# EugenHotaj/pytorch-generative

Hardware: NVIDIA H100
Metric: images/sec training step (ImageGPT CIFAR-10 32x32) (higher is better)
Workload: dtype bf16

## Files before the change

### pytorch_generative_b200/csrc/pg_attention.cu

```cuda
#include <stdlib.h>
#include <type_traits>

#include "../../include/pg_b200.h"
#include "pg_common.cuh"

namespace {

constexpr int MAX_S = 1024;
constexpr int MAX_D = 128;

struct AttnArgs {
  const bf16 *q, *k, *v, *o, *d_o;
  bf16 *out, *dq, *dk_out, *dv_out;
  int64_t ld_q, ld_k, ld_v, ld_o, ld_do, ld_dq, ld_dk, ld_dv;
  float* lse;
  const float* lse_in;
  float* delta;
  int N, S, H, dk, dv, strict;
  float scale;
};

__global__ void __launch_bounds__(128) attn_fwd_simt(const AttnArgs a) {
  extern __shared__ float sm[];
  const int lane = threadIdx.x & 31, w = threadIdx.x >> 5;
// ... 6 lines not shown
  const int h = (int)((gw / a.S) % a.H);
  const int n = (int)(gw / ((long long)a.S * a.H));
  const size_t row0 = (size_t)n * a.S;
  for (int d = lane; d < a.dk; d += 32) qs[d] = __bfloat162float(a.q[(row0 + i) * a.ld_q + h * a.dk + d]);
  __syncwarp();
  const int nkeys = a.strict ? i : i + 1;
  float m = -INFINITY;
  for (int j = lane; j < nkeys; j += 32) {
    const bf16* kr = a.k + (row0 + j) * a.ld_k + h * a.dk;
    float s = 0.f;
    for (int d = 0; d < a.dk; ++d) s = fmaf(qs[d], __bfloat162float(kr[d]), s);
    s *= a.scale;
    sc[j] = s;
    m = fmaxf(m, s);
  }
  m = warp_max(m);
  float l = 0.f;
  for (int j = lane; j < nkeys; j += 32) {
    const float p = __expf(sc[j] - m);
    sc[j] = p;
    l += p;
  }
  l = warp_sum(l);
  __syncwarp();
  const float inv = nkeys > 0 ? 1.f / l : 0.f;
  for (int d = lane; d < a.dv; d += 32) {
    float acc = 0.f;
    for (int j = 0; j < nkeys; ++j) acc = fmaf(sc[j], __bfloat162float(a.v[(row0 + j) * a.ld_v + h * a.dv + d]), acc);
    a.out[(row0 + i) * a.ld_o + h * a.dv + d] = __float2bfloat16(acc * inv);
  }
  if (lane == 0 && a.lse) a.lse[((size_t)n * a.H + h) * a.S + i] = nkeys > 0 ? m + __logf(l) : 0.f;
}

__global__ void attn_delta_kernel(const AttnArgs a) {
  const int lanes_per = a.dv / 8;
  const long long total = (long long)a.N * a.S * a.H * lanes_per;
  for (long long idx = (long long)blockIdx.x * blockDim.x + threadIdx.x; idx < total;
       idx += (long long)gridDim.x * blockDim.x) {
    const int sub = (int)(idx % lanes_per);
    const long long rh = idx / lanes_per;
    const int h = (int)(rh % a.H);
    const long long row = rh / a.H;
    const uint4 x = *reinterpret_cast<const uint4*>(a.d_o + row * a.ld_do + h * a.dv + sub * 8);
    const uint4 y = *reinterpret_cast<const uint4*>(a.o + row * a.ld_o + h * a.dv + sub * 8);
    const uint32_t xw[4] = {x.x, x.y, x.z, x.w}, yw[4] = {y.x, y.y, y.z, y.w};
    float s = 0.f;
#pragma unroll
    for (int t = 0; t < 4; ++t) {
      const float2 p = unpack_bf16x2(xw[t]), q = unpack_bf16x2(yw[t]);
      s = fmaf(p.x, q.x, fmaf(p.y, q.y, s));
    }
    for (int o = lanes_per >> 1; o > 0; o >>= 1) s += __shfl_xor_sync(0xffffffffu, s, o);
    if (sub == 0) {
      const int n = (int)(row / a.S), i = (int)(row % a.S);
      a.delta[((size_t)n * a.H + h) * a.S + i] = s;
    }
  }
}

__global__ void attn_delta_generic_kernel(const AttnArgs a) {
  const int lane = threadIdx.x & 31;
  const long long gw = ((long long)blockIdx.x * blockDim.x + threadIdx.x) >> 5;
  const long long total = (long long)a.N * a.H * a.S;
  if (gw >= total) return;
  const int i = (int)(gw % a.S);
  const int h = (int)((gw / a.S) % a.H);
  const int n = (int)(gw / ((long long)a.S * a.H));
  const size_t row = (size_t)n * a.S + i;
  float s = 0.f;
  for (int d = lane; d < a.dv; d += 32)
    s += __bfloat162float(a.d_o[row * a.ld_do + h * a.dv + d]) * __bfloat162float(a.o[row * a.ld_o + h * a.dv + d]);
  s = warp_sum(s);
  if (lane == 0) a.delta[((size_t)n * a.H + h) * a.S + i] = s;
}

__global__ void __launch_bounds__(128) attn_bwd_dq_simt(const AttnArgs a) {
  extern __shared__ float sm[];
  const int lane = threadIdx.x & 31, w = threadIdx.x >> 5;
  float* ds = sm + w * (MAX_S + 2 * MAX_D);
  float* qs = ds + MAX_S;
  float* dos = qs + MAX_D;
  const long long gw = (long long)blockIdx.x * 4 + w;
  const long long total = (long long)a.N * a.H * a.S;
  if (gw >= total) return;
// ... 187 lines not shown
  AttnArgs a = {};
  a.q = (const bf16*)q; a.k = (const bf16*)k; a.v = (const bf16*)v; a.out = (bf16*)o;
  a.ld_q = ld_q; a.ld_k = ld_k; a.ld_v = ld_v; a.ld_o = ld_o;
  a.lse = lse;
  a.N = N; a.S = S; a.H = H; a.dk = dk; a.dv = dv; a.strict = strict;
  a.scale = scale;
  if (impl == 1) {
    PG_REQUIRE(S <= MAX_S && dk <= MAX_D && dv <= MAX_D, "pg_causal_attn_fwd(simt): S<=%d, d<=%d", MAX_S, MAX_D);
    const long long total = (long long)N * H * S;
    const size_t smem = 4 * (MAX_S + MAX_D) * sizeof(float);
    attn_fwd_simt<<<(unsigned)((total + 3) / 4), 128, smem, stream>>>(a);
    return pg_check_launch("pg_causal_attn_fwd(simt)");
  }
  return attn_fwd_tc(a, stream);
}

extern "C" int pg_causal_attn_bwd(const void* q, int64_t ld_q, const void* k, int64_t ld_k, const void* v,
                                  int64_t ld_v, const void* o, int64_t ld_o, const void* d_o, int64_t ld_do,
                                  const float* lse, float* delta, float* dq_accum, void* dq, int64_t ld_dq, void* dk_,
                                  int64_t ld_dk, void* dv_, int64_t ld_dv, int N, int S, int H, int dk, int dv,
                                  float scale, int strict, int impl, void* stream_) {
  cudaStream_t stream = reinterpret_cast<cudaStream_t>(stream_);
  PG_REQUIRE(q && k && v && o && d_o && lse && delta && dq && dk_ && dv_, "pg_causal_attn_bwd: null argument");
  PG_REQUIRE(N > 0 && S > 0 && H > 0 && dk > 0 && dv > 0, "pg_causal_attn_bwd: empty problem");
  AttnArgs a = {};
  a.q = (const bf16*)q; a.k = (const bf16*)k; a.v = (const bf16*)v; a.o = (const bf16*)o; a.d_o = (const bf16*)d_o;
  a.dq = (bf16*)dq; a.dk_out = (bf16*)dk_; a.dv_out = (bf16*)dv_;
  a.ld_q = ld_q; a.ld_k = ld_k; a.ld_v = ld_v; a.ld_o = ld_o; a.ld_do = ld_do;
  a.ld_dq = ld_dq; a.ld_dk = ld_dk; a.ld_dv = ld_dv;
  a.lse_in = lse; a.delta = delta;
  a.N = N; a.S = S; a.H = H; a.dk = dk; a.dv = dv; a.strict = strict;
  a.scale = scale;
  (void)dq_accum;
  const long long total = (long long)N * H * S;
  const int lanes_per = dv / 8;
  const bool pow2 = dv % 8 == 0 && lanes_per >= 1 && lanes_per <= 32 && (lanes_per & (lanes_per - 1)) == 0;
  if (pow2 && ld_o % 8 == 0 && ld_do % 8 == 0 && (total * lanes_per) % 32 == 0) {
    long long blocks = (total * lanes_per + 255) / 256;
    if (blocks > (long long)pg_num_sms() * 32) blocks = (long long)pg_num_sms() * 32;
    attn_delta_kernel<<<(unsigned)blocks, 256, 0, stream>>>(a);
  } else {
    attn_delta_generic_kernel<<<(unsigned)((total * 32 + 255) / 256), 256, 0, stream>>>(a);
  }
  if (pg_check_launch("pg_causal_attn_bwd(delta)")) return 1;
  if (impl == 1) {
    PG_REQUIRE(S <= MAX_S && dk <= MAX_D && dv <= MAX_D, "pg_causal_attn_bwd(simt): S<=%d, d<=%d", MAX_S, MAX_D);
    const size_t smem_q = 4 * (MAX_S + 2 * MAX_D) * sizeof(float);
    const size_t smem_kv = 4 * (2 * MAX_S + 2 * MAX_D) * sizeof(float);
    attn_bwd_dq_simt<<<(unsigned)((total + 3) / 4), 128, smem_q, stream>>>(a);
    if (pg_check_launch("pg_causal_attn_bwd(dq simt)")) return 1;
    attn_bwd_dkv_simt<<<(unsigned)((total + 3) / 4), 128, smem_kv, stream>>>(a);
    return pg_check_launch("pg_causal_attn_bwd(dkv simt)");
  }
  return attn_bwd_tc(a, stream);
}

extern "C" int pg_attn_decode(const void* q, int64_t ld_q, const void* k_new, int64_t ld_kn, const void* v_new, int64_t ld_vn,
                              void* k_cache, int64_t ld_kc, void* v_cache, int64_t ld_vc, void* o, int64_t ld_o,
                              const int* pos_dev, int N, int S, int H, int dk, int dv, float scale, int strict,
                              void* stream_) {
  cudaStream_t stream = reinterpret_cast<cudaStream_t>(stream_);
  PG_REQUIRE(q && k_new && v_new && k_cache && v_cache && o && pos_dev, "pg_attn_decode: null argument");
  PG_REQUIRE(dk <= MAX_D && dv <= MAX_D, "pg_attn_decode: d<=%d", MAX_D);
  DecodeArgs a;
  a.q = (const bf16*)q; a.k_new = (const bf16*)k_new; a.v_new = (const bf16*)v_new;
  a.k_cache = (bf16*)k_cache; a.v_cache = (bf16*)v_cache; a.out = (bf16*)o;
  a.ld_q = ld_q; a.ld_kn = ld_kn; a.ld_vn = ld_vn; a.ld_kc = ld_kc; a.ld_vc = ld_vc; a.ld_o = ld_o;
  a.pos = pos_dev; a.N = N; a.S = S; a.H = H; a.dk = dk; a.dv = dv; a.strict = strict; a.scale = scale;
  a.part = nullptr;
  PG_REQUIRE(dk % 8 == 0 && ld_kc % 8 == 0, "pg_attn_decode: dk and the cache pitch must be multiples of 8");
  if (S <= MAX_S) {
    attn_decode_kernel<false><<<N * H, 128, 0, stream>>>(a);
    return pg_check_launch("pg_attn_decode");
  }
  const int splits = (S + MAX_S - 1) / MAX_S;
  if (pg_scratch((size_t)N * H * splits * (2 + dv) * sizeof(float), stream, &a.part)) return 1;
  attn_decode_kernel<true><<<dim3(N * H, splits), 128, 0, stream>>>(a);
  if (pg_check_launch("pg_attn_decode(split)")) return 1;
  attn_decode_merge_kernel<<<N * H, 128, 0, stream>>>(a, splits);
  return pg_check_launch("pg_attn_decode(merge)");
}
```

### pytorch_generative_b200/csrc/pg_attention_tc.cuh

```cuda
#pragma once

namespace {

constexpr int AT = 128;
constexpr int ATOM_BYTES = AT * 128;
constexpr int BQ = 64;
constexpr int QATOM_BYTES = BQ * 128;
constexpr int ATTN_THREADS = 384;
constexpr int ATTN_PRODUCER_REGS = 24, ATTN_CONSUMER_REGS = 240;
constexpr int ATTN_SMEM_LIMIT = 227 * 1024;
constexpr int ATTN_BAR_BYTES = 128;
constexpr int ATTN_TURN_BAR = 1;

constexpr int attn_stages(int fixed, int stage) {
  const int fit = (ATTN_SMEM_LIMIT - ATTN_BAR_BYTES - fixed) / stage;
  return fit < 4 ? fit : 4;
}

__device__ __forceinline__ void attn_turn_wait(int wg, int it) {
  if (wg | it) named_bar_sync(ATTN_TURN_BAR + wg, 256);
}
__device__ __forceinline__ void attn_turn_pass(int wg, int it, int niter) {
  if (wg == 0 || it + 1 < niter) named_bar_arrive(ATTN_TURN_BAR + (wg ^ 1), 256);
}

__device__ __forceinline__ float fast_exp2(float x) {
  float y;
  asm("ex2.approx.ftz.f32 %0, %1;" : "=f"(y) : "f"(x));
  return y;
}
__device__ __forceinline__ float quad_max(float v) {
  v = fmaxf(v, __shfl_xor_sync(0xffffffffu, v, 1));
  return fmaxf(v, __shfl_xor_sync(0xffffffffu, v, 2));
}
__device__ __forceinline__ float quad_sum(float v) {
  v += __shfl_xor_sync(0xffffffffu, v, 1);
  return v + __shfl_xor_sync(0xffffffffu, v, 2);
}

struct AttnTmaps {
  CUtensorMap q, k, v, d_o;
};

template <int DK, int DV>
__global__ void __launch_bounds__(ATTN_THREADS, 1)
attn_fwd_tc_kernel(const __grid_constant__ AttnTmaps tm, const AttnArgs a, const int T) {
  constexpr int K_BYTES = DK * 256;
  constexpr int V_BYTES = DV * 256;
  constexpr int ST = attn_stages(K_BYTES, K_BYTES + V_BYTES);
  extern __shared__ __align__(1024) uint8_t smem[];
  uint8_t* sQ = smem;
  uint8_t* sK = sQ + K_BYTES;
  uint8_t* sV = sK + ST * K_BYTES;
  uint64_t* bars = reinterpret_cast<uint64_t*>(sV + ST * V_BYTES);
  uint64_t* q_full = bars;
  uint64_t* kv_full = bars + 1;
  uint64_t* kv_empty = bars + 1 + ST;

  const int warp = threadIdx.x >> 5, lane = threadIdx.x & 31;
  const int nh = blockIdx.x / T;
  const int i = T - 1 - blockIdx.x % T;
  const int n = nh / a.H, h = nh % a.H;
  const int ntiles = i + 1;

  if (threadIdx.x == 0) {
    if (smem_u32(smem) & 1023u) __trap();
    mbar_init(q_full, 1);
    for (int s = 0; s < ST; ++s) {
      mbar_init(&kv_full[s], 1);
      mbar_init(&kv_empty[s], 8);
    }
    fence_barrier_init();
    fence_proxy_async_smem();
  }
  __syncthreads();
// ... 91 lines not shown
#pragma unroll
      for (int kk = 0; kk < 8; ++kk) wgmma_frag_a(S, kk, pa[kk]);
      const uint64_t v_d = wgmma_desc_sw128(smem_u32(sV + st * V_BYTES), ATOM_BYTES, 1024);
      wgmma_fence();
#pragma unroll
      for (int kk = 0; kk < 8; ++kk) Wgmma<DV>::template rs<1>(O, pa[kk], v_d + kk * 128, 1u);
      wgmma_commit();
      wgmma_wait<0>();
      wgmma_hold(O);
      __syncwarp();
      if (lane == 0) mbar_arrive(&kv_empty[st]);
    }
    l0 = quad_sum(l0);
    l1 = quad_sum(l1);
#pragma unroll
    for (int half = 0; half < 2; ++half) {
      const int qi = half ? qi1 : qi0;
      const float l = half ? l1 : l0, m = half ? m1 : m0;
      if (qi < a.S) {
        const float inv = l > 0.f ? 1.f / l : 0.f;
        bf16* orow = a.out + ((size_t)n * a.S + qi) * a.ld_o + h * DV + 2 * (lane & 3);
#pragma unroll
        for (int d = 0; d < DV / 8; ++d)
          *reinterpret_cast<uint32_t*>(orow + 8 * d) = pack_bf16x2(O[4 * d + 2 * half] * inv, O[4 * d + 2 * half + 1] * inv);
        if ((lane & 3) == 0) a.lse[((size_t)n * a.H + h) * a.S + qi] = l > 0.f ? m * a.scale + __logf(l) : 0.f;
      }
    }
  }
}

template <int DK, int DV>
__global__ void __launch_bounds__(ATTN_THREADS, 1)
attn_bwd_tc_kernel(const __grid_constant__ AttnTmaps tm, const AttnArgs a, const int T) {
  constexpr int K_BYTES = DK * 256;
  constexpr int V_BYTES = DV * 256;
  constexpr int Q_BYTES = DK * 128;
  constexpr int DO_BYTES = DV * 128;
  constexpr int STAT_BYTES = 2 * BQ * 4;
  constexpr int ST = attn_stages(K_BYTES + V_BYTES, Q_BYTES + DO_BYTES + STAT_BYTES);
  extern __shared__ __align__(1024) uint8_t smem[];
  uint8_t* sK = smem;
  uint8_t* sV = sK + K_BYTES;
  uint8_t* sQ = sV + V_BYTES;
  uint8_t* sdO = sQ + ST * Q_BYTES;
  float* sStat = reinterpret_cast<float*>(sdO + ST * DO_BYTES);
  uint64_t* bars = reinterpret_cast<uint64_t*>(sStat + ST * 2 * BQ);
  uint64_t* kv_full = bars;
  uint64_t* qdo_full = bars + 1;
  uint64_t* qdo_empty = bars + 1 + ST;

  const int warp = threadIdx.x >> 5, lane = threadIdx.x & 31;
  const int nh = blockIdx.x % (a.N * a.H);
  const int j = blockIdx.x / (a.N * a.H);
  const int n = nh / a.H, h = nh % a.H;
  const int it0 = j * (AT / BQ);
  const int niter = (a.S + BQ - 1) / BQ - it0;

  if (threadIdx.x == 0) {
    if (smem_u32(smem) & 1023u) __trap();
    mbar_init(kv_full, 1);
    for (int s = 0; s < ST; ++s) {
      mbar_init(&qdo_full[s], 1);
      mbar_init(&qdo_empty[s], 8);
    }
    fence_barrier_init();
    fence_proxy_async_smem();
  }
  __syncthreads();

  if (warp < 4) {
    setmaxnreg_dec<ATTN_PRODUCER_REGS>();
    if (warp == 0) {
      mbar_arrive_expect_tx_w(kv_full, K_BYTES + V_BYTES);
#pragma unroll
      for (int c = 0; c < DK / 64; ++c) tma_load_3d_w(sK + c * ATOM_BYTES, &tm.k, kv_full, h * DK + c * 64, j * AT, n);
#pragma unroll
      for (int v = 0; v < DV / 64; ++v) tma_load_3d_w(sV + v * ATOM_BYTES, &tm.v, kv_full, h * DV + v * 64, j * AT, n);
      const float* lse_nh = a.lse_in + ((size_t)n * a.H + h) * a.S;
      const float* delta_nh = a.delta + ((size_t)n * a.H + h) * a.S;
      for (int it = 0; it < niter; ++it) {
        const int st = it % ST, i = it0 + it;
        const int qa = i * BQ + lane, qb = qa + 32;
        const float lse_a = qa < a.S ? lse_nh[qa] * 1.4426950408889634f : 0.f;
        const float lse_b = qb < a.S ? lse_nh[qb] * 1.4426950408889634f : 0.f;
        const float delta_a = qa < a.S ? delta_nh[qa] : 0.f, delta_b = qb < a.S ? delta_nh[qb] : 0.f;
        mbar_wait(&qdo_empty[st], ((it / ST) & 1) ^ 1);
        float* stat = sStat + st * 2 * BQ;
        stat[lane] = lse_a;
        stat[lane + 32] = lse_b;
        stat[BQ + lane] = delta_a;
        stat[BQ + lane + 32] = delta_b;
        __syncwarp();
        mbar_arrive_expect_tx_w(&qdo_full[st], Q_BYTES + DO_BYTES);
#pragma unroll
        for (int c = 0; c < DK / 64; ++c)
          tma_load_3d_w(sQ + st * Q_BYTES + c * QATOM_BYTES, &tm.q, &qdo_full[st], h * DK + c * 64, i * BQ, n);
#pragma unroll
        for (int v = 0; v < DV / 64; ++v)
          tma_load_3d_w(sdO + st * DO_BYTES + v * QATOM_BYTES, &tm.d_o, &qdo_full[st], h * DV + v * 64, i * BQ, n);
      }
    }
  } else {
    setmaxnreg_inc<ATTN_CONSUMER_REGS>();
    const int wg = (warp >> 2) - 1, wi = warp & 3;
    const int kr = wg * 64 + wi * 16 + (lane >> 2);
    const int kj0 = j * AT + kr, kj1 = kj0 + 8;
    const float sl2 = a.scale * 1.4426950408889634f;
    float dV[DV / 2], dK[DK / 2];
#pragma unroll
    for (int d = 0; d < DV / 2; ++d) dV[d] = 0.f;
#pragma unroll
    for (int d = 0; d < DK / 2; ++d) dK[d] = 0.f;
    const uint32_t k_rows = smem_u32(sK) + wg * 64 * 128;
    const uint32_t v_rows = smem_u32(sV) + wg * 64 * 128;
    mbar_wait(kv_full, 0);
    for (int it = 0; it < niter; ++it) {
      const int st = it % ST;
      const int q0 = (it0 + it) * BQ;
      mbar_wait(&qdo_full[st], (it / ST) & 1);
      const uint32_t q_addr = smem_u32(sQ + st * Q_BYTES), do_addr = smem_u32(sdO + st * DO_BYTES);
      const float* stat = sStat + st * 2 * BQ + 2 * (lane & 3);
      float sT[32], dpT[32];
      attn_turn_wait(wg, it);
      wgmma_fence();
#pragma unroll
      for (int kk = 0; kk < DK / 16; ++kk)
        Wgmma<64>::ss<0, 0>(sT, wgmma_desc_sw128(k_rows + (kk >> 2) * ATOM_BYTES + (kk & 3) * 32, 16, 1024),
                            wgmma_desc_sw128(q_addr + (kk >> 2) * QATOM_BYTES + (kk & 3) * 32, 16, 1024),
                            kk > 0 ? 1u : 0u);
#pragma unroll
      for (int kk = 0; kk < DV / 16; ++kk)
        Wgmma<64>::ss<0, 0>(dpT, wgmma_desc_sw128(v_rows + (kk >> 2) * ATOM_BYTES + (kk & 3) * 32, 16, 1024),
                            wgmma_desc_sw128(do_addr + (kk >> 2) * QATOM_BYTES + (kk & 3) * 32, 16, 1024),
                            kk > 0 ? 1u : 0u);
      wgmma_commit();
      attn_turn_pass(wg, it, niter);
      wgmma_wait<0>();
      wgmma_hold(sT);
      wgmma_hold(dpT);
#pragma unroll
      for (int jj = 0; jj < 8; ++jj) {
        const float2 lse2_pair = *reinterpret_cast<const float2*>(stat + 8 * jj);
        const float2 delta_pair = *reinterpret_cast<const float2*>(stat + BQ + 8 * jj);
#pragma unroll
        for (int e = 0; e < 2; ++e) {
          const int qi = q0 + 8 * jj + 2 * (lane & 3) + e;
          const float lse2 = e ? lse2_pair.y : lse2_pair.x, delta = e ? delta_pair.y : delta_pair.x;
          const int qlim = qi < a.S ? qi - a.strict : -1;
          const float p0 = kj0 <= qlim ? fast_exp2(fmaf(sT[4 * jj + e], sl2, -lse2)) : 0.f;
          const float p1 = kj1 <= qlim ? fast_exp2(fmaf(sT[4 * jj + 2 + e], sl2, -lse2)) : 0.f;
          sT[4 * jj + e] = p0;
          sT[4 * jj + 2 + e] = p1;
          dpT[4 * jj + e] = p0 * (dpT[4 * jj + e] - delta);
          dpT[4 * jj + 2 + e] = p1 * (dpT[4 * jj + 2 + e] - delta);
        }
      }
      uint32_t pa[4][4], dsa[4][4];
#pragma unroll
      for (int kk = 0; kk < 4; ++kk) {
        wgmma_frag_a(sT, kk, pa[kk]);
        wgmma_frag_a(dpT, kk, dsa[kk]);
      }
      wgmma_fence();
#pragma unroll
      for (int kk = 0; kk < 4; ++kk)
        Wgmma<DV>::template rs<1>(dV, pa[kk], wgmma_desc_sw128(do_addr + kk * 2048, QATOM_BYTES, 1024), 1u);
#pragma unroll
      for (int kk = 0; kk < 4; ++kk)
        Wgmma<DK>::template rs<1>(dK, dsa[kk], wgmma_desc_sw128(q_addr + kk * 2048, QATOM_BYTES, 1024), 1u);
      wgmma_commit();
      wgmma_wait<0>();
      wgmma_hold(dV);
      wgmma_hold(dK);
      __syncwarp();
      if (lane == 0) mbar_arrive(&qdo_empty[st]);
    }
#pragma unroll
    for (int half = 0; half < 2; ++half) {
      const int kj = half ? kj1 : kj0;
      if (kj < a.S) {
        bf16* dvrow = a.dv_out + ((size_t)n * a.S + kj) * a.ld_dv + h * DV + 2 * (lane & 3);
#pragma unroll
        for (int d = 0; d < DV / 8; ++d)
          *reinterpret_cast<uint32_t*>(dvrow + 8 * d) = pack_bf16x2(dV[4 * d + 2 * half], dV[4 * d + 2 * half + 1]);
        bf16* dkrow = a.dk_out + ((size_t)n * a.S + kj) * a.ld_dk + h * DK + 2 * (lane & 3);
#pragma unroll
        for (int d = 0; d < DK / 8; ++d)
          *reinterpret_cast<uint32_t*>(dkrow + 8 * d) =
              pack_bf16x2(dK[4 * d + 2 * half] * a.scale, dK[4 * d + 2 * half + 1] * a.scale);
      }
    }
  }
}

template <int DK, int DV>
__global__ void __launch_bounds__(ATTN_THREADS, 1)
attn_dq_tc_kernel(const __grid_constant__ AttnTmaps tm, const AttnArgs a, const int T) {
  constexpr int K_BYTES = DK * 256;
  constexpr int V_BYTES = DV * 256;
  constexpr int KS = DK == 64 ? AT : 64;
  constexpr int ST = attn_stages(K_BYTES + V_BYTES, K_BYTES + V_BYTES);
  extern __shared__ __align__(1024) uint8_t smem[];
  uint8_t* sQ = smem;
  uint8_t* sdO = sQ + K_BYTES;
  uint8_t* sK = sdO + V_BYTES;
  uint8_t* sV = sK + ST * K_BYTES;
  uint64_t* bars = reinterpret_cast<uint64_t*>(sV + ST * V_BYTES);
  uint64_t* q_full = bars;
  uint64_t* kv_full = bars + 1;
  uint64_t* kv_empty = bars + 1 + ST;

  const int warp = threadIdx.x >> 5, lane = threadIdx.x & 31;
  const int nh = blockIdx.x / T;
  const int i = T - 1 - blockIdx.x % T;
  const int n = nh / a.H, h = nh % a.H;
  const int ntiles = i + 1;

  if (threadIdx.x == 0) {
    if (smem_u32(smem) & 1023u) __trap();
    mbar_init(q_full, 1);
    for (int s = 0; s < ST; ++s) {
      mbar_init(&kv_full[s], 1);
      mbar_init(&kv_empty[s], 8);
    }
    fence_barrier_init();
    fence_proxy_async_smem();
  }
  __syncthreads();

  if (warp < 4) {
    setmaxnreg_dec<ATTN_PRODUCER_REGS>();
    if (warp == 0) {
      mbar_arrive_expect_tx_w(q_full, K_BYTES + V_BYTES);
#pragma unroll
      for (int c = 0; c < DK / 64; ++c) tma_load_3d_w(sQ + c * ATOM_BYTES, &tm.q, q_full, h * DK + c * 64, i * AT, n);
#pragma unroll
      for (int v = 0; v < DV / 64; ++v) tma_load_3d_w(sdO + v * ATOM_BYTES, &tm.d_o, q_full, h * DV + v * 64, i * AT, n);
      for (int jj = 0; jj < ntiles; ++jj) {
        const int st = jj % ST;
        mbar_wait(&kv_empty[st], ((jj / ST) & 1) ^ 1);
        mbar_arrive_expect_tx_w(&kv_full[st], K_BYTES + V_BYTES);
#pragma unroll
        for (int c = 0; c < DK / 64; ++c)
          tma_load_3d_w(sK + st * K_BYTES + c * ATOM_BYTES, &tm.k, &kv_full[st], h * DK + c * 64, jj * AT, n);
#pragma unroll
        for (int v = 0; v < DV / 64; ++v)
          tma_load_3d_w(sV + st * V_BYTES + v * ATOM_BYTES, &tm.v, &kv_full[st], h * DV + v * 64, jj * AT, n);
      }
    }
  } else {
    setmaxnreg_inc<ATTN_CONSUMER_REGS>();
    const int wg = (warp >> 2) - 1;
    const int r0 = wg * 64 + (warp & 3) * 16 + (lane >> 2);
    const int qi0 = i * AT + r0, qi1 = qi0 + 8;
    const size_t stat_base = ((size_t)n * a.H + h) * a.S;
    const float sl2 = a.scale * 1.4426950408889634f;
    const int qlim0 = qi0 < a.S ? qi0 - a.strict : -1, qlim1 = qi1 < a.S ? qi1 - a.strict : -1;
    const float lse0 = qi0 < a.S ? a.lse_in[stat_base + qi0] * 1.4426950408889634f : 0.f;
    const float lse1 = qi1 < a.S ? a.lse_in[stat_base + qi1] * 1.4426950408889634f : 0.f;
    const float delta0 = qi0 < a.S ? a.delta[stat_base + qi0] : 0.f;
    const float delta1 = qi1 < a.S ? a.delta[stat_base + qi1] : 0.f;
    float dQ[DK / 2];
#pragma unroll
    for (int d = 0; d < DK / 2; ++d) dQ[d] = 0.f;
    const uint32_t q_rows = smem_u32(sQ) + wg * 64 * 128, do_rows = smem_u32(sdO) + wg * 64 * 128;
    mbar_wait(q_full, 0);
    for (int j = 0; j < ntiles; ++j) {
      const int st = j % ST;
      mbar_wait(&kv_full[st], (j / ST) & 1);
      const uint32_t k_tile = smem_u32(sK + st * K_BYTES), v_tile = smem_u32(sV + st * V_BYTES);
#pragma unroll
      for (int ks = 0; ks < AT / KS; ++ks) {
        const uint32_t k_addr = k_tile + ks * KS * 128, v_addr = v_tile + ks * KS * 128;
        float S[KS / 2], dP[KS / 2];
        attn_turn_wait(wg, j * (AT / KS) + ks);
        wgmma_fence();
#pragma unroll
        for (int kk = 0; kk < DK / 16; ++kk)
          Wgmma<KS>::template ss<0, 0>(S, wgmma_desc_sw128(q_rows + (kk >> 2) * ATOM_BYTES + (kk & 3) * 32, 16, 1024),
                                       wgmma_desc_sw128(k_addr + (kk >> 2) * ATOM_BYTES + (kk & 3) * 32, 16, 1024),
                                       kk > 0 ? 1u : 0u);
#pragma unroll
        for (int kk = 0; kk < DV / 16; ++kk)
          Wgmma<KS>::template ss<0, 0>(dP, wgmma_desc_sw128(do_rows + (kk >> 2) * ATOM_BYTES + (kk & 3) * 32, 16, 1024),
                                       wgmma_desc_sw128(v_addr + (kk >> 2) * ATOM_BYTES + (kk & 3) * 32, 16, 1024),
                                       kk > 0 ? 1u : 0u);
        wgmma_commit();
        attn_turn_pass(wg, j * (AT / KS) + ks, ntiles * (AT / KS));
        wgmma_wait<0>();
        wgmma_hold(S);
        wgmma_hold(dP);
        const int k0 = j * AT + ks * KS + 2 * (lane & 3);
#pragma unroll
        for (int jj = 0; jj < KS / 8; ++jj) {
#pragma unroll
          for (int e = 0; e < 2; ++e) {
            const int kj = k0 + 8 * jj + e;
            const float p0 = kj <= qlim0 ? fast_exp2(fmaf(S[4 * jj + e], sl2, -lse0)) : 0.f;
            const float p1 = kj <= qlim1 ? fast_exp2(fmaf(S[4 * jj + 2 + e], sl2, -lse1)) : 0.f;
            dP[4 * jj + e] = p0 * (dP[4 * jj + e] - delta0);
            dP[4 * jj + 2 + e] = p1 * (dP[4 * jj + 2 + e] - delta1);
          }
        }
        uint32_t dsa[KS / 16][4];
#pragma unroll
        for (int kk = 0; kk < KS / 16; ++kk) wgmma_frag_a(dP, kk, dsa[kk]);
        wgmma_fence();
#pragma unroll
        for (int kk = 0; kk < KS / 16; ++kk)
          Wgmma<DK>::template rs<1>(dQ, dsa[kk], wgmma_desc_sw128(k_addr + kk * 2048, ATOM_BYTES, 1024), 1u);
        wgmma_commit();
        wgmma_wait<0>();
        wgmma_hold(dQ);
      }
      __syncwarp();
      if (lane == 0) mbar_arrive(&kv_empty[st]);
    }
#pragma unroll
    for (int half = 0; half < 2; ++half) {
      const int qi = half ? qi1 : qi0;
      if (qi < a.S) {
// ... 2 lines not shown
        for (int d = 0; d < DK / 8; ++d)
          *reinterpret_cast<uint32_t*>(drow + 8 * d) =
              pack_bf16x2(dQ[4 * d + 2 * half] * a.scale, dQ[4 * d + 2 * half + 1] * a.scale);
      }
    }
  }
}

int make_attn_map(CUtensorMap* out, const bf16* base, int64_t ld, int width, int S, int N, int rows) {
  uint64_t dims[3] = {(uint64_t)width, (uint64_t)S, (uint64_t)N};
  uint64_t strides[2] = {(uint64_t)ld * 2, (uint64_t)S * (uint64_t)ld * 2};
  uint32_t box[3] = {64, (uint32_t)rows, 1};
  return pg_make_tmap_nd_bf16(out, base, 3, dims, strides, box, 1);
}

int attn_check_tc(const AttnArgs& a, const char* who) {
  PG_REQUIRE(a.dk == 64 || a.dk == 128, "%s: tensor-core path needs q/k head slots of 64 or 128 columns (dk=%d)", who,
             a.dk);
  PG_REQUIRE(a.dv == 64 || a.dv == 128, "%s: tensor-core path needs v head slots of 64 or 128 columns (dv=%d)", who,
             a.dv);
  return 0;
}

template <int DK, int DV>
int launch_fwd(const AttnTmaps& tm, const AttnArgs& a, int T, unsigned grid, cudaStream_t stream) {
  constexpr int SMEM = DK * 256 + attn_stages(DK * 256, (DK + DV) * 256) * (DK + DV) * 256 + ATTN_BAR_BYTES;
  static_assert(SMEM <= ATTN_SMEM_LIMIT, "attn_fwd_tc_kernel: shared memory");
  PG_CUDA(cudaFuncSetAttribute(attn_fwd_tc_kernel<DK, DV>, cudaFuncAttributeMaxDynamicSharedMemorySize, SMEM));
  attn_fwd_tc_kernel<DK, DV><<<grid, ATTN_THREADS, SMEM, stream>>>(tm, a, T);
  return 0;
}
template <int DK, int DV>
int launch_bwd(const AttnTmaps& tm, const AttnArgs& a, int T, unsigned grid, cudaStream_t stream) {
  constexpr int STAGE = (DK + DV) * 128 + 2 * BQ * 4;
  constexpr int SMEM = (DK + DV) * 256 + attn_stages((DK + DV) * 256, STAGE) * STAGE + ATTN_BAR_BYTES;
  static_assert(SMEM <= ATTN_SMEM_LIMIT, "attn_bwd_tc_kernel: shared memory");
  PG_CUDA(cudaFuncSetAttribute(attn_bwd_tc_kernel<DK, DV>, cudaFuncAttributeMaxDynamicSharedMemorySize, SMEM));
  attn_bwd_tc_kernel<DK, DV><<<grid, ATTN_THREADS, SMEM, stream>>>(tm, a, T);
  return 0;
}
template <int DK, int DV>
int launch_dq(const AttnTmaps& tm, const AttnArgs& a, int T, unsigned grid, cudaStream_t stream) {
  constexpr int SMEM = (1 + attn_stages((DK + DV) * 256, (DK + DV) * 256)) * (DK + DV) * 256 + ATTN_BAR_BYTES;
  static_assert(SMEM <= ATTN_SMEM_LIMIT, "attn_dq_tc_kernel: shared memory");
  PG_CUDA(cudaFuncSetAttribute(attn_dq_tc_kernel<DK, DV>, cudaFuncAttributeMaxDynamicSharedMemorySize, SMEM));
  attn_dq_tc_kernel<DK, DV><<<grid, ATTN_THREADS, SMEM, stream>>>(tm, a, T);
  return 0;
}

using AttnLaunch = int (*)(const AttnTmaps&, const AttnArgs&, int, unsigned, cudaStream_t);
constexpr AttnLaunch kFwd[2][2] = {{launch_fwd<64, 64>, launch_fwd<64, 128>}, {launch_fwd<128, 64>, launch_fwd<128, 128>}};
constexpr AttnLaunch kBwd[2][2] = {{launch_bwd<64, 64>, launch_bwd<64, 128>}, {launch_bwd<128, 64>, launch_bwd<128, 128>}};
constexpr AttnLaunch kDq[2][2] = {{launch_dq<64, 64>, launch_dq<64, 128>}, {launch_dq<128, 64>, launch_dq<128, 128>}};

int attn_fwd_tc(const AttnArgs& a, cudaStream_t stream) {
  if (attn_check_tc(a, "pg_causal_attn_fwd")) return 1;
  PG_REQUIRE(a.ld_o % 8 == 0, "pg_causal_attn_fwd: output pitch must be a multiple of 8");
  AttnTmaps tm;
  if (make_attn_map(&tm.q, a.q, a.ld_q, a.H * a.dk, a.S, a.N, AT)) return 1;
  if (make_attn_map(&tm.k, a.k, a.ld_k, a.H * a.dk, a.S, a.N, AT)) return 1;
  if (make_attn_map(&tm.v, a.v, a.ld_v, a.H * a.dv, a.S, a.N, AT)) return 1;
  tm.d_o = tm.v;
  const int T = (a.S + AT - 1) / AT;
  const unsigned grid = (unsigned)(a.N * a.H * T);
  if (kFwd[a.dk == 128][a.dv == 128](tm, a, T, grid, stream)) return 1;
  return pg_check_launch("pg_causal_attn_fwd(wgmma)");
}

int attn_bwd_tc(const AttnArgs& a, cudaStream_t stream) {
  if (attn_check_tc(a, "pg_causal_attn_bwd")) return 1;
  PG_REQUIRE(a.ld_dq % 8 == 0 && a.ld_dk % 8 == 0 && a.ld_dv % 8 == 0, "pg_causal_attn_bwd: pitches must be multiples of 8");
  AttnTmaps tm;
  if (make_attn_map(&tm.q, a.q, a.ld_q, a.H * a.dk, a.S, a.N, BQ)) return 1;
  if (make_attn_map(&tm.k, a.k, a.ld_k, a.H * a.dk, a.S, a.N, AT)) return 1;
  if (make_attn_map(&tm.v, a.v, a.ld_v, a.H * a.dv, a.S, a.N, AT)) return 1;
  if (make_attn_map(&tm.d_o, a.d_o, a.ld_do, a.H * a.dv, a.S, a.N, BQ)) return 1;
  const int T = (a.S + AT - 1) / AT;
  const unsigned grid = (unsigned)(a.N * a.H * T);
  if (kBwd[a.dk == 128][a.dv == 128](tm, a, T, grid, stream)) return 1;
  if (pg_check_launch("pg_causal_attn_bwd(wgmma dk/dv)")) return 1;
  if (make_attn_map(&tm.q, a.q, a.ld_q, a.H * a.dk, a.S, a.N, AT)) return 1;
  if (make_attn_map(&tm.d_o, a.d_o, a.ld_do, a.H * a.dv, a.S, a.N, AT)) return 1;
  if (kDq[a.dk == 128][a.dv == 128](tm, a, T, grid, stream)) return 1;
  return pg_check_launch("pg_causal_attn_bwd(wgmma dq)");
}

}
```

Measured before the change: 537.0.

## Fuse delta computation into dQ kernel and enlarge backward query tile

Drops the separate delta kernel on the tensor-core backward path. The dQ kernel now TMA-loads O alongside dO, computes rowwise dot(dO,O) from swizzled shared memory while the first wgmma runs, and writes delta out for the dK/dV kernel, which is reordered to run after dQ. The dK/dV kernel also uses a 128-row query tile when dk=dv=64, skips masking on fully unmasked tiles, and for 64-row tiles issues the dV wgmma before computing dS. The cost is more shared memory in dQ (which can mean fewer stages) and more register pressure from the larger tile.

New measurement: 547.7, median of 6. 2.0% higher.

```diff
diff --git a/pytorch_generative_b200/csrc/pg_attention.cu b/pytorch_generative_b200/csrc/pg_attention.cu
--- a/pytorch_generative_b200/csrc/pg_attention.cu
+++ b/pytorch_generative_b200/csrc/pg_attention.cu
@@ -62,6 +62,17 @@
   if (lane == 0 && a.lse) a.lse[((size_t)n * a.H + h) * a.S + i] = nkeys > 0 ? m + __logf(l) : 0.f;
 }
 
+__device__ __forceinline__ float attn_delta_dot8(const uint4 x, const uint4 y) {
+  const uint32_t xw[4] = {x.x, x.y, x.z, x.w}, yw[4] = {y.x, y.y, y.z, y.w};
+  float s = 0.f;
+#pragma unroll
+  for (int t = 0; t < 4; ++t) {
+    const float2 p = unpack_bf16x2(xw[t]), q = unpack_bf16x2(yw[t]);
+    s = fmaf(p.x, q.x, fmaf(p.y, q.y, s));
+  }
+  return s;
+}
+
 __global__ void attn_delta_kernel(const AttnArgs a) {
   const int lanes_per = a.dv / 8;
   const long long total = (long long)a.N * a.S * a.H * lanes_per;
@@ -71,15 +82,8 @@
     const long long rh = idx / lanes_per;
     const int h = (int)(rh % a.H);
     const long long row = rh / a.H;
-    const uint4 x = *reinterpret_cast<const uint4*>(a.d_o + row * a.ld_do + h * a.dv + sub * 8);
-    const uint4 y = *reinterpret_cast<const uint4*>(a.o + row * a.ld_o + h * a.dv + sub * 8);
-    const uint32_t xw[4] = {x.x, x.y, x.z, x.w}, yw[4] = {y.x, y.y, y.z, y.w};
-    float s = 0.f;
-#pragma unroll
-    for (int t = 0; t < 4; ++t) {
-      const float2 p = unpack_bf16x2(xw[t]), q = unpack_bf16x2(yw[t]);
-      s = fmaf(p.x, q.x, fmaf(p.y, q.y, s));
-    }
+    float s = attn_delta_dot8(*reinterpret_cast<const uint4*>(a.d_o + row * a.ld_do + h * a.dv + sub * 8),
+                              *reinterpret_cast<const uint4*>(a.o + row * a.ld_o + h * a.dv + sub * 8));
     for (int o = lanes_per >> 1; o > 0; o >>= 1) s += __shfl_xor_sync(0xffffffffu, s, o);
     if (sub == 0) {
       const int n = (int)(row / a.S), i = (int)(row % a.S);
@@ -333,6 +337,7 @@
   a.N = N; a.S = S; a.H = H; a.dk = dk; a.dv = dv; a.strict = strict;
   a.scale = scale;
   (void)dq_accum;
+  if (impl != 1) return attn_bwd_tc(a, stream);
   const long long total = (long long)N * H * S;
   const int lanes_per = dv / 8;
   const bool pow2 = dv % 8 == 0 && lanes_per >= 1 && lanes_per <= 32 && (lanes_per & (lanes_per - 1)) == 0;
@@ -344,16 +349,13 @@
     attn_delta_generic_kernel<<<(unsigned)((total * 32 + 255) / 256), 256, 0, stream>>>(a);
   }
   if (pg_check_launch("pg_causal_attn_bwd(delta)")) return 1;
-  if (impl == 1) {
-    PG_REQUIRE(S <= MAX_S && dk <= MAX_D && dv <= MAX_D, "pg_causal_attn_bwd(simt): S<=%d, d<=%d", MAX_S, MAX_D);
-    const size_t smem_q = 4 * (MAX_S + 2 * MAX_D) * sizeof(float);
-    const size_t smem_kv = 4 * (2 * MAX_S + 2 * MAX_D) * sizeof(float);
-    attn_bwd_dq_simt<<<(unsigned)((total + 3) / 4), 128, smem_q, stream>>>(a);
-    if (pg_check_launch("pg_causal_attn_bwd(dq simt)")) return 1;
-    attn_bwd_dkv_simt<<<(unsigned)((total + 3) / 4), 128, smem_kv, stream>>>(a);
-    return pg_check_launch("pg_causal_attn_bwd(dkv simt)");
-  }
-  return attn_bwd_tc(a, stream);
+  PG_REQUIRE(S <= MAX_S && dk <= MAX_D && dv <= MAX_D, "pg_causal_attn_bwd(simt): S<=%d, d<=%d", MAX_S, MAX_D);
+  const size_t smem_q = 4 * (MAX_S + 2 * MAX_D) * sizeof(float);
+  const size_t smem_kv = 4 * (2 * MAX_S + 2 * MAX_D) * sizeof(float);
+  attn_bwd_dq_simt<<<(unsigned)((total + 3) / 4), 128, smem_q, stream>>>(a);
+  if (pg_check_launch("pg_causal_attn_bwd(dq simt)")) return 1;
+  attn_bwd_dkv_simt<<<(unsigned)((total + 3) / 4), 128, smem_kv, stream>>>(a);
+  return pg_check_launch("pg_causal_attn_bwd(dkv simt)");
 }
 
 extern "C" int pg_attn_decode(const void* q, int64_t ld_q, const void* k_new, int64_t ld_kn, const void* v_new, int64_t ld_vn,
diff --git a/pytorch_generative_b200/csrc/pg_attention_tc.cuh b/pytorch_generative_b200/csrc/pg_attention_tc.cuh
--- a/pytorch_generative_b200/csrc/pg_attention_tc.cuh
+++ b/pytorch_generative_b200/csrc/pg_attention_tc.cuh
@@ -4,13 +4,14 @@
 
 constexpr int AT = 128;
 constexpr int ATOM_BYTES = AT * 128;
-constexpr int BQ = 64;
-constexpr int QATOM_BYTES = BQ * 128;
 constexpr int ATTN_THREADS = 384;
 constexpr int ATTN_PRODUCER_REGS = 24, ATTN_CONSUMER_REGS = 240;
 constexpr int ATTN_SMEM_LIMIT = 227 * 1024;
 constexpr int ATTN_BAR_BYTES = 128;
 constexpr int ATTN_TURN_BAR = 1;
+constexpr int ATTN_DELTA_BAR = 3;
+
+constexpr int attn_bwd_qtile(int dk, int dv) { return dk == 64 && dv == 64 ? 128 : 64; }
 
 constexpr int attn_stages(int fixed, int stage) {
   const int fit = (ATTN_SMEM_LIMIT - ATTN_BAR_BYTES - fixed) / stage;
@@ -39,8 +40,44 @@
 }
 
 struct AttnTmaps {
-  CUtensorMap q, k, v, d_o;
+  CUtensorMap q, k, v, d_o, o;
 };
+
+template <bool MASK, int R>
+__device__ __forceinline__ void attn_bwd_p(float (&sT)[R], const float* stat, int q0, int kj0, int kj1, float sl2,
+                                           const AttnArgs& a, int lane) {
+#pragma unroll
+  for (int jj = 0; jj < R / 4; ++jj) {
+    const float2 lse2_pair = *reinterpret_cast<const float2*>(stat + 8 * jj);
+#pragma unroll
+    for (int e = 0; e < 2; ++e) {
+      const float lse2 = e ? lse2_pair.y : lse2_pair.x;
+      float p0 = fast_exp2(fmaf(sT[4 * jj + e], sl2, -lse2));
+      float p1 = fast_exp2(fmaf(sT[4 * jj + 2 + e], sl2, -lse2));
+      if (MASK) {
+        const int qi = q0 + 8 * jj + 2 * (lane & 3) + e;
+        const int qlim = qi < a.S ? qi - a.strict : -1;
+        if (kj0 > qlim) p0 = 0.f;
+        if (kj1 > qlim) p1 = 0.f;
+      }
+      sT[4 * jj + e] = p0;
+      sT[4 * jj + 2 + e] = p1;
+    }
+  }
+}
+template <int R>
+__device__ __forceinline__ void attn_bwd_ds(const float (&pT)[R], float (&dpT)[R], const float* stat) {
+#pragma unroll
+  for (int jj = 0; jj < R / 4; ++jj) {
+    const float2 delta_pair = *reinterpret_cast<const float2*>(stat + 2 * R + 8 * jj);
+#pragma unroll
+    for (int e = 0; e < 2; ++e) {
+      const float delta = e ? delta_pair.y : delta_pair.x;
+      dpT[4 * jj + e] = pT[4 * jj + e] * (dpT[4 * jj + e] - delta);
+      dpT[4 * jj + 2 + e] = pT[4 * jj + 2 + e] * (dpT[4 * jj + 2 + e] - delta);
+    }
+  }
+}
 
 template <int DK, int DV>
 __global__ void __launch_bounds__(ATTN_THREADS, 1)
@@ -198,11 +235,13 @@
 template <int DK, int DV>
 __global__ void __launch_bounds__(ATTN_THREADS, 1)
 attn_bwd_tc_kernel(const __grid_constant__ AttnTmaps tm, const AttnArgs a, const int T) {
+  constexpr int QT = attn_bwd_qtile(DK, DV);
+  constexpr int QATOM = QT * 128;
   constexpr int K_BYTES = DK * 256;
   constexpr int V_BYTES = DV * 256;
-  constexpr int Q_BYTES = DK * 128;
-  constexpr int DO_BYTES = DV * 128;
-  constexpr int STAT_BYTES = 2 * BQ * 4;
+  constexpr int Q_BYTES = DK * QT * 2;
+  constexpr int DO_BYTES = DV * QT * 2;
+  constexpr int STAT_BYTES = 2 * QT * 4;
   constexpr int ST = attn_stages(K_BYTES + V_BYTES, Q_BYTES + DO_BYTES + STAT_BYTES);
   extern __shared__ __align__(1024) uint8_t smem[];
   uint8_t* sK = smem;
@@ -210,7 +249,7 @@
   uint8_t* sQ = sV + V_BYTES;
   uint8_t* sdO = sQ + ST * Q_BYTES;
   float* sStat = reinterpret_cast<float*>(sdO + ST * DO_BYTES);
-  uint64_t* bars = reinterpret_cast<uint64_t*>(sStat + ST * 2 * BQ);
+  uint64_t* bars = reinterpret_cast<uint64_t*>(sStat + ST * 2 * QT);
   uint64_t* kv_full = bars;
   uint64_t* qdo_full = bars + 1;
   uint64_t* qdo_empty = bars + 1 + ST;
@@ -219,8 +258,8 @@
   const int nh = blockIdx.x % (a.N * a.H);
   const int j = blockIdx.x / (a.N * a.H);
   const int n = nh / a.H, h = nh % a.H;
-  const int it0 = j * (AT / BQ);
-  const int niter = (a.S + BQ - 1) / BQ - it0;
+  const int it0 = j * (AT / QT);
+  const int niter = (a.S + QT - 1) / QT - it0;
 
   if (threadIdx.x == 0) {
     if (smem_u32(smem) & 1023u) __trap();
@@ -246,24 +285,28 @@
       const float* delta_nh = a.delta + ((size_t)n * a.H + h) * a.S;
       for (int it = 0; it < niter; ++it) {
         const int st = it % ST, i = it0 + it;
-        const int qa = i * BQ + lane, qb = qa + 32;
-        const float lse_a = qa < a.S ? lse_nh[qa] * 1.4426950408889634f : 0.f;
-        const float lse_b = qb < a.S ? lse_nh[qb] * 1.4426950408889634f : 0.f;
-        const float delta_a = qa < a.S ? delta_nh[qa] : 0.f, delta_b = qb < a.S ? delta_nh[qb] : 0.f;
+        float lse2[QT / 32], dlt[QT / 32];
+#pragma unroll
+        for (int r = 0; r < QT / 32; ++r) {
+          const int q = i * QT + 32 * r + lane;
+          lse2[r] = q < a.S ? lse_nh[q] * 1.4426950408889634f : 0.f;
+          dlt[r] = q < a.S ? delta_nh[q] : 0.f;
+        }
         mbar_wait(&qdo_empty[st], ((it / ST) & 1) ^ 1);
-        float* stat = sStat + st * 2 * BQ;
-        stat[lane] = lse_a;
-        stat[lane + 32] = lse_b;
-        stat[BQ + lane] = delta_a;
-        stat[BQ + lane + 32] = delta_b;
+        float* stat = sStat + st * 2 * QT;
+#pragma unroll
+        for (int r = 0; r < QT / 32; ++r) {
+          stat[32 * r + lane] = lse2[r];
+          stat[QT + 32 * r + lane] = dlt[r];
+        }
         __syncwarp();
         mbar_arrive_expect_tx_w(&qdo_full[st], Q_BYTES + DO_BYTES);
 #pragma unroll
         for (int c = 0; c < DK / 64; ++c)
-          tma_load_3d_w(sQ + st * Q_BYTES + c * QATOM_BYTES, &tm.q, &qdo_full[st], h * DK + c * 64, i * BQ, n);
+          tma_load_3d_w(sQ + st * Q_BYTES + c * QATOM, &tm.q, &qdo_full[st], h * DK + c * 64, i * QT, n);
 #pragma unroll
         for (int v = 0; v < DV / 64; ++v)
-          tma_load_3d_w(sdO + st * DO_BYTES + v * QATOM_BYTES, &tm.d_o, &qdo_full[st], h * DV + v * 64, i * BQ, n);
+          tma_load_3d_w(sdO + st * DO_BYTES + v * QATOM, &tm.d_o, &qdo_full[st], h * DV + v * 64, i * QT, n);
       }
     }
   } else {
@@ -282,58 +325,54 @@
     mbar_wait(kv_full, 0);
     for (int it = 0; it < niter; ++it) {
       const int st = it % ST;
-      const int q0 = (it0 + it) * BQ;
+      const int q0 = (it0 + it) * QT;
       mbar_wait(&qdo_full[st], (it / ST) & 1);
       const uint32_t q_addr = smem_u32(sQ + st * Q_BYTES), do_addr = smem_u32(sdO + st * DO_BYTES);
-      const float* stat = sStat + st * 2 * BQ + 2 * (lane & 3);
-      float sT[32], dpT[32];
+      const float* stat = sStat + st * 2 * QT + 2 * (lane & 3);
+      float sT[QT / 2], dpT[QT / 2];
       attn_turn_wait(wg, it);
       wgmma_fence();
 #pragma unroll
       for (int kk = 0; kk < DK / 16; ++kk)
-        Wgmma<64>::ss<0, 0>(sT, wgmma_desc_sw128(k_rows + (kk >> 2) * ATOM_BYTES + (kk & 3) * 32, 16, 1024),
-                            wgmma_desc_sw128(q_addr + (kk >> 2) * QATOM_BYTES + (kk & 3) * 32, 16, 1024),
-                            kk > 0 ? 1u : 0u);
+        Wgmma<QT>::template ss<0, 0>(sT, wgmma_desc_sw128(k_rows + (kk >> 2) * ATOM_BYTES + (kk & 3) * 32, 16, 1024),
+                                     wgmma_desc_sw128(q_addr + (kk >> 2) * QATOM + (kk & 3) * 32, 16, 1024),
+                                     kk > 0 ? 1u : 0u);
 #pragma unroll
       for (int kk = 0; kk < DV / 16; ++kk)
-        Wgmma<64>::ss<0, 0>(dpT, wgmma_desc_sw128(v_rows + (kk >> 2) * ATOM_BYTES + (kk & 3) * 32, 16, 1024),
-                            wgmma_desc_sw128(do_addr + (kk >> 2) * QATOM_BYTES + (kk & 3) * 32, 16, 1024),
-                            kk > 0 ? 1u : 0u);
+        Wgmma<QT>::template ss<0, 0>(dpT, wgmma_desc_sw128(v_rows + (kk >> 2) * ATOM_BYTES + (kk & 3) * 32, 16, 1024),
+                                     wgmma_desc_sw128(do_addr + (kk >> 2) * QATOM + (kk & 3) * 32, 16, 1024),
+                                     kk > 0 ? 1u : 0u);
       wgmma_commit();
       attn_turn_pass(wg, it, niter);
       wgmma_wait<0>();
       wgmma_hold(sT);
       wgmma_hold(dpT);
-#pragma unroll
-      for (int jj = 0; jj < 8; ++jj) {
-        const float2 lse2_pair = *reinterpret_cast<const float2*>(stat + 8 * jj);
-        const float2 delta_pair = *reinterpret_cast<const float2*>(stat + BQ + 8 * jj);
-#pragma unroll
-        for (int e = 0; e < 2; ++e) {
-          const int qi = q0 + 8 * jj + 2 * (lane & 3) + e;
-          const float lse2 = e ? lse2_pair.y : lse2_pair.x, delta = e ? delta_pair.y : delta_pair.x;
-          const int qlim = qi < a.S ? qi - a.strict : -1;
-          const float p0 = kj0 <= qlim ? fast_exp2(fmaf(sT[4 * jj + e], sl2, -lse2)) : 0.f;
-          const float p1 = kj1 <= qlim ? fast_exp2(fmaf(sT[4 * jj + 2 + e], sl2, -lse2)) : 0.f;
-          sT[4 * jj + e] = p0;
-          sT[4 * jj + 2 + e] = p1;
-          dpT[4 * jj + e] = p0 * (dpT[4 * jj + e] - delta);
-          dpT[4 * jj + 2 + e] = p1 * (dpT[4 * jj + 2 + e] - delta);
-        }
-      }
-      uint32_t pa[4][4], dsa[4][4];
-#pragma unroll
-      for (int kk = 0; kk < 4; ++kk) {
-        wgmma_frag_a(sT, kk, pa[kk]);
-        wgmma_frag_a(dpT, kk, dsa[kk]);
+      if (q0 < (j + 1) * AT || q0 + QT > a.S)
+        attn_bwd_p<true>(sT, stat, q0, kj0, kj1, sl2, a, lane);
+      else
+        attn_bwd_p<false>(sT, stat, q0, kj0, kj1, sl2, a, lane);
+      constexpr bool DV_FIRST = QT == 64;
+      uint32_t pa[QT / 16][4], dsa[QT / 16][4];
+      if (!DV_FIRST) attn_bwd_ds(sT, dpT, stat);
+#pragma unroll
+      for (int kk = 0; kk < QT / 16; ++kk) wgmma_frag_a(sT, kk, pa[kk]);
+      if (!DV_FIRST) {
+#pragma unroll
+        for (int kk = 0; kk < QT / 16; ++kk) wgmma_frag_a(dpT, kk, dsa[kk]);
       }
       wgmma_fence();
 #pragma unroll
-      for (int kk = 0; kk < 4; ++kk)
-        Wgmma<DV>::template rs<1>(dV, pa[kk], wgmma_desc_sw128(do_addr + kk * 2048, QATOM_BYTES, 1024), 1u);
-#pragma unroll
-      for (int kk = 0; kk < 4; ++kk)
-        Wgmma<DK>::template rs<1>(dK, dsa[kk], wgmma_desc_sw128(q_addr + kk * 2048, QATOM_BYTES, 1024), 1u);
+      for (int kk = 0; kk < QT / 16; ++kk)
+        Wgmma<DV>::template rs<1>(dV, pa[kk], wgmma_desc_sw128(do_addr + kk * 2048, QATOM, 1024), 1u);
+      if (DV_FIRST) {
+        attn_bwd_ds(sT, dpT, stat);
+#pragma unroll
+        for (int kk = 0; kk < QT / 16; ++kk) wgmma_frag_a(dpT, kk, dsa[kk]);
+        wgmma_fence();
+      }
+#pragma unroll
+      for (int kk = 0; kk < QT / 16; ++kk)
+        Wgmma<DK>::template rs<1>(dK, dsa[kk], wgmma_desc_sw128(q_addr + kk * 2048, QATOM, 1024), 1u);
       wgmma_commit();
       wgmma_wait<0>();
       wgmma_hold(dV);
@@ -365,16 +404,18 @@
   constexpr int K_BYTES = DK * 256;
   constexpr int V_BYTES = DV * 256;
   constexpr int KS = DK == 64 ? AT : 64;
-  constexpr int ST = attn_stages(K_BYTES + V_BYTES, K_BYTES + V_BYTES);
+  constexpr int ST = attn_stages(K_BYTES + 2 * V_BYTES + AT * 4, K_BYTES + V_BYTES);
   extern __shared__ __align__(1024) uint8_t smem[];
   uint8_t* sQ = smem;
   uint8_t* sdO = sQ + K_BYTES;
-  uint8_t* sK = sdO + V_BYTES;
+  uint8_t* sO = sdO + V_BYTES;
+  uint8_t* sK = sO + V_BYTES;
   uint8_t* sV = sK + ST * K_BYTES;
   uint64_t* bars = reinterpret_cast<uint64_t*>(sV + ST * V_BYTES);
   uint64_t* q_full = bars;
   uint64_t* kv_full = bars + 1;
   uint64_t* kv_empty = bars + 1 + ST;
+  float* sDelta = reinterpret_cast<float*>(reinterpret_cast<uint8_t*>(bars) + ATTN_BAR_BYTES);
 
   const int warp = threadIdx.x >> 5, lane = threadIdx.x & 31;
   const int nh = blockIdx.x / T;
@@ -397,11 +438,14 @@
   if (warp < 4) {
     setmaxnreg_dec<ATTN_PRODUCER_REGS>();
     if (warp == 0) {
-      mbar_arrive_expect_tx_w(q_full, K_BYTES + V_BYTES);
+      mbar_arrive_expect_tx_w(q_full, K_BYTES + 2 * V_BYTES);
 #pragma unroll
       for (int c = 0; c < DK / 64; ++c) tma_load_3d_w(sQ + c * ATOM_BYTES, &tm.q, q_full, h * DK + c * 64, i * AT, n);
 #pragma unroll
-      for (int v = 0; v < DV / 64; ++v) tma_load_3d_w(sdO + v * ATOM_BYTES, &tm.d_o, q_full, h * DV + v * 64, i * AT, n);
+      for (int v = 0; v < DV / 64; ++v) {
+        tma_load_3d_w(sdO + v * ATOM_BYTES, &tm.d_o, q_full, h * DV + v * 64, i * AT, n);
+        tma_load_3d_w(sO + v * ATOM_BYTES, &tm.o, q_full, h * DV + v * 64, i * AT, n);
+      }
       for (int jj = 0; jj < ntiles; ++jj) {
         const int st = jj % ST;
         mbar_wait(&kv_empty[st], ((jj / ST) & 1) ^ 1);
@@ -424,13 +468,12 @@
     const int qlim0 = qi0 < a.S ? qi0 - a.strict : -1, qlim1 = qi1 < a.S ? qi1 - a.strict : -1;
     const float lse0 = qi0 < a.S ? a.lse_in[stat_base + qi0] * 1.4426950408889634f : 0.f;
     const float lse1 = qi1 < a.S ? a.lse_in[stat_base + qi1] * 1.4426950408889634f : 0.f;
-    const float delta0 = qi0 < a.S ? a.delta[stat_base + qi0] : 0.f;
-    const float delta1 = qi1 < a.S ? a.delta[stat_base + qi1] : 0.f;
+    mbar_wait(q_full, 0);
+    float delta0, delta1;
     float dQ[DK / 2];
 #pragma unroll
     for (int d = 0; d < DK / 2; ++d) dQ[d] = 0.f;
     const uint32_t q_rows = smem_u32(sQ) + wg * 64 * 128, do_rows = smem_u32(sdO) + wg * 64 * 128;
-    mbar_wait(q_full, 0);
     for (int j = 0; j < ntiles; ++j) {
       const int st = j % ST;
       mbar_wait(&kv_full[st], (j / ST) & 1);
@@ -453,6 +496,25 @@
                                        kk > 0 ? 1u : 0u);
         wgmma_commit();
         attn_turn_pass(wg, j * (AT / KS) + ks, ntiles * (AT / KS));
+        if (j == 0 && ks == 0) {
+          constexpr int DLANES = DV / 8;
+#pragma unroll
+          for (int pass = 0; pass < DV / 16; ++pass) {
+            const int idx = pass * 128 + (int)(threadIdx.x & 127);
+            const int r = wg * 64 + idx / DLANES, sub = idx % DLANES;
+            const int off = (sub >> 3) * ATOM_BYTES + r * 128 + (((sub & 7) ^ (r & 7)) << 4);
+            float s = attn_delta_dot8(*reinterpret_cast<const uint4*>(sdO + off), *reinterpret_cast<const uint4*>(sO + off));
+#pragma unroll
+            for (int o = DLANES >> 1; o > 0; o >>= 1) s += __shfl_xor_sync(0xffffffffu, s, o);
+            if (sub == 0) {
+              sDelta[r] = s;
+              if (i * AT + r < a.S) a.delta[stat_base + i * AT + r] = s;
+            }
+          }
+          named_bar_sync(ATTN_DELTA_BAR + wg, 128);
+          delta0 = sDelta[r0];
+          delta1 = sDelta[r0 + 8];
+        }
         wgmma_wait<0>();
         wgmma_hold(S);
         wgmma_hold(dP);
@@ -521,7 +583,8 @@
 }
 template <int DK, int DV>
 int launch_bwd(const AttnTmaps& tm, const AttnArgs& a, int T, unsigned grid, cudaStream_t stream) {
-  constexpr int STAGE = (DK + DV) * 128 + 2 * BQ * 4;
+  constexpr int QT = attn_bwd_qtile(DK, DV);
+  constexpr int STAGE = (DK + DV) * QT * 2 + 2 * QT * 4;
   constexpr int SMEM = (DK + DV) * 256 + attn_stages((DK + DV) * 256, STAGE) * STAGE + ATTN_BAR_BYTES;
   static_assert(SMEM <= ATTN_SMEM_LIMIT, "attn_bwd_tc_kernel: shared memory");
   PG_CUDA(cudaFuncSetAttribute(attn_bwd_tc_kernel<DK, DV>, cudaFuncAttributeMaxDynamicSharedMemorySize, SMEM));
@@ -530,7 +593,8 @@
 }
 template <int DK, int DV>
 int launch_dq(const AttnTmaps& tm, const AttnArgs& a, int T, unsigned grid, cudaStream_t stream) {
-  constexpr int SMEM = (1 + attn_stages((DK + DV) * 256, (DK + DV) * 256)) * (DK + DV) * 256 + ATTN_BAR_BYTES;
+  constexpr int SMEM = (1 + attn_stages((DK + 2 * DV) * 256 + AT * 4, (DK + DV) * 256)) * (DK + DV) * 256 + DV * 256 +
+                       ATTN_BAR_BYTES + AT * 4;
   static_assert(SMEM <= ATTN_SMEM_LIMIT, "attn_dq_tc_kernel: shared memory");
   PG_CUDA(cudaFuncSetAttribute(attn_dq_tc_kernel<DK, DV>, cudaFuncAttributeMaxDynamicSharedMemorySize, SMEM));
   attn_dq_tc_kernel<DK, DV><<<grid, ATTN_THREADS, SMEM, stream>>>(tm, a, T);
@@ -549,7 +613,7 @@
   if (make_attn_map(&tm.q, a.q, a.ld_q, a.H * a.dk, a.S, a.N, AT)) return 1;
   if (make_attn_map(&tm.k, a.k, a.ld_k, a.H * a.dk, a.S, a.N, AT)) return 1;
   if (make_attn_map(&tm.v, a.v, a.ld_v, a.H * a.dv, a.S, a.N, AT)) return 1;
-  tm.d_o = tm.v;
+  tm.d_o = tm.o = tm.v;
   const int T = (a.S + AT - 1) / AT;
   const unsigned grid = (unsigned)(a.N * a.H * T);
   if (kFwd[a.dk == 128][a.dv == 128](tm, a, T, grid, stream)) return 1;
@@ -558,20 +622,25 @@
 
 int attn_bwd_tc(const AttnArgs& a, cudaStream_t stream) {
   if (attn_check_tc(a, "pg_causal_attn_bwd")) return 1;
-  PG_REQUIRE(a.ld_dq % 8 == 0 && a.ld_dk % 8 == 0 && a.ld_dv % 8 == 0, "pg_causal_attn_bwd: pitches must be multiples of 8");
+  PG_REQUIRE(a.ld_dq % 8 == 0 && a.ld_dk % 8 == 0 && a.ld_dv % 8 == 0 && a.ld_o % 8 == 0 && a.ld_do % 8 == 0,
+             "pg_causal_attn_bwd: pitches must be multiples of 8");
   AttnTmaps tm;
-  if (make_attn_map(&tm.q, a.q, a.ld_q, a.H * a.dk, a.S, a.N, BQ)) return 1;
+  if (make_attn_map(&tm.q, a.q, a.ld_q, a.H * a.dk, a.S, a.N, AT)) return 1;
   if (make_attn_map(&tm.k, a.k, a.ld_k, a.H * a.dk, a.S, a.N, AT)) return 1;
   if (make_attn_map(&tm.v, a.v, a.ld_v, a.H * a.dv, a.S, a.N, AT)) return 1;
-  if (make_attn_map(&tm.d_o, a.d_o, a.ld_do, a.H * a.dv, a.S, a.N, BQ)) return 1;
+  if (make_attn_map(&tm.d_o, a.d_o, a.ld_do, a.H * a.dv, a.S, a.N, AT)) return 1;
+  if (make_attn_map(&tm.o, a.o, a.ld_o, a.H * a.dv, a.S, a.N, AT)) return 1;
   const int T = (a.S + AT - 1) / AT;
   const unsigned grid = (unsigned)(a.N * a.H * T);
+  if (kDq[a.dk == 128][a.dv == 128](tm, a, T, grid, stream)) return 1;
+  if (pg_check_launch("pg_causal_attn_bwd(wgmma dq)")) return 1;
+  const int qt = attn_bwd_qtile(a.dk, a.dv);
+  if (qt != AT) {
+    if (make_attn_map(&tm.q, a.q, a.ld_q, a.H * a.dk, a.S, a.N, qt)) return 1;
+    if (make_attn_map(&tm.d_o, a.d_o, a.ld_do, a.H * a.dv, a.S, a.N, qt)) return 1;
+  }
   if (kBwd[a.dk == 128][a.dv == 128](tm, a, T, grid, stream)) return 1;
-  if (pg_check_launch("pg_causal_attn_bwd(wgmma dk/dv)")) return 1;
-  if (make_attn_map(&tm.q, a.q, a.ld_q, a.H * a.dk, a.S, a.N, AT)) return 1;
-  if (make_attn_map(&tm.d_o, a.d_o, a.ld_do, a.H * a.dv, a.S, a.N, AT)) return 1;
-  if (kDq[a.dk == 128][a.dv == 128](tm, a, T, grid, stream)) return 1;
-  return pg_check_launch("pg_causal_attn_bwd(wgmma dq)");
-}
-
-}
+  return pg_check_launch("pg_causal_attn_bwd(wgmma dk/dv)");
+}
+
+}
```
